# thrill/thrill

Hardware: AMD Instinct MI355X
Metric: TeraSort keys/sec (100-byte recs) (higher is better)
Workload: dtype u8; 1 GPU; terasort_10GiB_100B; records=107374182, record_bytes=100, seed=0x7421, parallelism=dp1

## Files before the change

include/thrill_amd.h:

```cpp
#ifndef THRILL_AMD_H
#define THRILL_AMD_H

#include <stdint.h>

#ifdef __cplusplus
extern "C" {
#endif

typedef struct t9_context t9_context;

int t9_create(t9_context** out, int device, int rank, int world, void* comm);
int t9_destroy(t9_context* ctx);
const char* t9_version(void);

int t9_comm_id_size(void);
int t9_comm_id(void* out_id);
int t9_comm_init(t9_context* ctx, const void* id);

int t9_gen_u64(t9_context* ctx, uint64_t* d_out, uint64_t index0, uint64_t n,
               uint64_t seed, void* stream);
int t9_gen_records(t9_context* ctx, uint8_t* d_out, uint64_t index0,
                   uint64_t n, uint64_t seed, void* stream);


uint64_t t9_sort_u64_workspace(uint64_t n);
int t9_sort_u64(t9_context* ctx, uint64_t* d_keys, uint64_t n,
                void* d_workspace, void* stream);

uint64_t t9_sort_pairs_workspace(uint64_t n);
int t9_sort_pairs_u64_u32(t9_context* ctx, uint64_t* d_keys,
                          uint32_t* d_vals, uint64_t n, void* d_workspace,
                          void* stream);

int t9_extract_key64(t9_context* ctx, const uint8_t* d_recs, uint64_t n,
                     uint32_t rec_size, uint32_t key_off, uint64_t* d_keys,
                     uint32_t* d_idx, void* stream);

int t9_extract_key64_le(t9_context* ctx, const uint8_t* d_recs, uint64_t n,
                        uint32_t rec_size, uint32_t key_off,
                        uint64_t* d_keys, uint32_t* d_idx, void* stream);

int t9_gather_records(t9_context* ctx, const uint8_t* d_recs,
                      const uint32_t* d_idx, uint64_t n, uint32_t rec_size,
                      uint8_t* d_out, void* stream);

uint64_t t9_sort_records_workspace(uint64_t n, uint32_t rec_size);
int t9_sort_records(t9_context* ctx, const uint8_t* d_in, uint8_t* d_out,
                    uint64_t n, uint32_t rec_size, uint32_t key_len,
                    void* d_workspace, void* stream);

int t9_sort_records_keyle(t9_context* ctx, const uint8_t* d_in,
                          uint8_t* d_out, uint64_t n, uint32_t rec_size,
                          void* d_workspace, void* stream);

int t9_sort_last_schedule(const t9_context* ctx);

int t9_sort_last_tiecount(const t9_context* ctx);


int t9_classify_u64(t9_context* ctx, const uint64_t* d_keys, uint64_t n,
                    uint64_t gidx0, const uint64_t* d_spl_keys,
                    const uint64_t* d_spl_idx, uint32_t p,
                    uint32_t* d_bucket, uint64_t* d_counts, void* stream);

int t9_classify_rec(t9_context* ctx, const uint8_t* d_recs,
                    const uint64_t* d_k64, uint64_t n, uint64_t gidx0,
                    const uint8_t* d_spl_recs, const uint64_t* d_spl_k64,
                    const uint64_t* d_spl_idx, uint32_t p, uint32_t rec_size,
                    uint32_t* d_bucket, uint64_t* d_counts, void* stream);

uint64_t t9_partition_idx_workspace(uint64_t n);
int t9_partition_idx(t9_context* ctx, const uint32_t* d_bucket, uint64_t n,
                     uint32_t p, uint32_t* d_perm, uint64_t* d_offsets,
                     void* d_workspace, void* stream);

int t9_alltoall(t9_context* ctx, const void* d_send,
                const uint64_t* send_counts, const uint64_t* send_displs,
                void* d_recv, const uint64_t* recv_counts,
                const uint64_t* recv_displs, uint64_t elem_size,
                void* stream);

int t9_hash_bucket(t9_context* ctx, const uint64_t* d_keys, uint64_t n,
                   uint64_t salt, uint32_t p, uint32_t* d_bucket,
                   uint64_t* d_counts, void* stream);

int t9_reduce_init(t9_context* ctx, uint64_t* d_table, uint64_t capacity,
                   void* stream);
int t9_reduce_build(t9_context* ctx, const uint64_t* d_keys,
                    const uint64_t* d_vals, uint64_t n,
                    uint64_t* d_table, uint64_t capacity, uint64_t salt,
// ... 128 lines not shown
```

thrill_amd/csrc/t9_api.cpp:

```cpp

#include "t9_common.h"

#include <rccl/rccl.h>

#include <cstdlib>
#include <cstring>
#include <new>

extern "C" {

const char* t9_version(void) { return "thrill_amd 0.1 (gfx950)"; }

int t9_create(t9_context** out, int device, int rank, int world,
              void* comm) {
    if (!out || world < 1 || rank < 0 || rank >= world) return T9_EINVAL;
    HIP_TRY(hipSetDevice(device));
    t9_context* ctx = new (std::nothrow) t9_context;
    if (!ctx) return T9_ENOMEM;
    ctx->device = device;
    ctx->rank = rank;
    ctx->world = world;
    ctx->comm = comm;
    ctx->owns_comm = 0;
    ctx->ov_stream = nullptr;
    for (int i = 0; i <= T9_OVERLAP_MAXK; ++i) ctx->ov_ev[i] = nullptr;
    ctx->ov_ready = 0;
    ctx->last_schedule = 0;
    ctx->last_tiecount = 0;
    *out = ctx;
    return T9_OK;
}

int t9_destroy(t9_context* ctx) {
    if (ctx && ctx->comm && ctx->owns_comm)
        ncclCommDestroy((ncclComm_t)ctx->comm);
    if (ctx) {
        if (ctx->ov_stream) {
            (void)hipStreamSynchronize(ctx->ov_stream);
            (void)hipStreamDestroy(ctx->ov_stream);
        }
        for (int i = 0; i <= T9_OVERLAP_MAXK; ++i)
            if (ctx->ov_ev[i]) (void)hipEventDestroy(ctx->ov_ev[i]);
    }
    delete ctx;
    return T9_OK;
}

int t9i_overlap_init(t9_context* ctx) {
    if (!ctx) return T9_EINVAL;
    if (ctx->ov_ready) return T9_OK;
    HIP_TRY(hipSetDevice(ctx->device));
    if (!ctx->ov_stream)
        HIP_TRY(hipStreamCreateWithFlags(&ctx->ov_stream,
                                         hipStreamNonBlocking));
    for (int i = 0; i <= T9_OVERLAP_MAXK; ++i)
        if (!ctx->ov_ev[i])
            HIP_TRY(hipEventCreateWithFlags(&ctx->ov_ev[i],
                                            hipEventDisableTiming));
    ctx->ov_ready = 1;
    return T9_OK;
}

int t9_sort_last_schedule(const t9_context* ctx) {
    return ctx ? ctx->last_schedule : T9_EINVAL;
}

int t9_sort_last_tiecount(const t9_context* ctx) {
    return ctx ? ctx->last_tiecount : T9_EINVAL;
}


int t9_comm_id_size(void) { return (int)sizeof(ncclUniqueId); }

int t9_comm_id(void* out_id) {
    if (!out_id) return T9_EINVAL;
    ncclResult_t rc = ncclGetUniqueId((ncclUniqueId*)out_id);
    if (rc != ncclSuccess) {
        fprintf(stderr, "t9_comm_id: %s\n", ncclGetErrorString(rc));
        return T9_EIO;
    }
    return T9_OK;
}

int t9_comm_init(t9_context* ctx, const void* id) {
    if (!ctx || !id) return T9_EINVAL;
    if (ctx->comm) return T9_EINVAL;
    HIP_TRY(hipSetDevice(ctx->device));
    ncclComm_t comm = nullptr;
    ncclResult_t rc = ncclCommInitRank(&comm, ctx->world,
                                       *(const ncclUniqueId*)id, ctx->rank);
    if (rc != ncclSuccess) {
        fprintf(stderr, "t9_comm_init: rank %d/%d: %s\n", ctx->rank,
                ctx->world, ncclGetErrorString(rc));
        return T9_EIO;
    }
    ctx->comm = comm;
    ctx->owns_comm = 1;
    return T9_OK;
}

int t9_alltoall(t9_context* ctx, const void* d_send, const u64* send_counts,
// ... 58 lines not shown
```

thrill_amd/csrc/t9_bitonic.h:

```cpp
#pragma once
#include "t9_common.h"

__device__ inline void t9_ce_xor(u64& c, u32& v, u32 lanemask, bool lower,
                                 bool asc) {
    const u64 oc = __shfl_xor(c, lanemask);
    const u32 ov = __shfl_xor(v, lanemask);
    if ((c > oc) == (lower == asc)) { c = oc; v = ov; }
}

template <int SUBMAX, int BLOCK, bool HAS_VAL>
__global__ __launch_bounds__(BLOCK, 2) void k_bitonic_sort_sub(
    u64* __restrict__ keys, u32* __restrict__ vals,
    const u32* __restrict__ sub_start, const u32* __restrict__ sub_n) {
    constexpr int E = SUBMAX / BLOCK;
    static_assert(E == 4, "mapping assumes 4 elements per thread");
    __shared__ u64 s_c[SUBMAX];
    __shared__ u32 s_v[HAS_VAL ? SUBMAX : 1];
    __shared__ u32 s_differ;

    const u32 sb = blockIdx.x;
    const u32 ns = sub_n[sb];
    if (ns <= 1 || ns > (u32)SUBMAX) return;
    const u32 gbase = sub_start[sb];
    const u32 tid = threadIdx.x, lane = tid & 63;
// ... 88 lines not shown
        }
    }
}

typedef unsigned long long t9_u64x2 __attribute__((ext_vector_type(2)));

__device__ __forceinline__ u32 t9_w16_phys(u32 e) {
    return e ^ (((e >> 4) & 7u) << 1);
}

__device__ __forceinline__ void t9_w16_row_store(u64* lc, u32 row,
                                                 const u64 (&c)[16]) {
    const u32 base = row * 16 + ((row & 7u) << 1);
#pragma unroll
    for (int k = 0; k < 8; ++k) {
        t9_u64x2 v2;
        v2.x = c[2 * k];
        v2.y = c[2 * k + 1];
        *(t9_u64x2*)&lc[base ^ ((u32)k << 1)] = v2;
    }
}

__device__ __forceinline__ void t9_w16_row_load(const u64* lc, u32 row,
                                                u64 (&c)[16]) {
    const u32 base = row * 16 + ((row & 7u) << 1);
#pragma unroll
    for (int k = 0; k < 8; ++k) {
        const t9_u64x2 v2 = *(const t9_u64x2*)&lc[base ^ ((u32)k << 1)];
        c[2 * k] = v2.x;
        c[2 * k + 1] = v2.y;
    }
}

template <int NSORT, int BLOCK, bool HAS_VAL, bool REC>
__global__ __launch_bounds__(BLOCK, 2) void k_wave16_sort_sub(
    u64* __restrict__ keys, u32* __restrict__ vals,
    const u32* __restrict__ sub_start, const u32* __restrict__ sub_n,
    u32* __restrict__ ntied) {
    constexpr int E = NSORT / BLOCK;
    static_assert(E == 16, "wave16 mapping: 16 elements per lane");
    static_assert(HAS_VAL || !REC, "the tie count rides the pair sort");
    constexpr int ROUNDS = (NSORT == 1024) ? 6 : (NSORT == 2048) ? 7 : 8;
    __shared__ __attribute__((aligned(16))) u64 lc[NSORT];
    __shared__ u32 s_differ;
    __shared__ u32 s_ntie;

    const u32 sb = blockIdx.x;
    const u32 ns = sub_n[sb];
    if (ns <= 1 || ns > (u32)NSORT) return;
    const u32 gbase = sub_start[sb];
    const u32 lane = threadIdx.x;
    const u32 e0 = lane * E;

    if (lane == 0) { s_differ = 0; s_ntie = 0; }
    __syncthreads();

    const u64 mask48 = 0x0000FFFFFFFFFFFFull;
    const u64 high16 = keys[gbase] & ~mask48;
    const u64 ref48 = keys[gbase] & mask48;

    u64 c[E];
    u32 differ = 0;
    u64* const kb = keys + gbase;
    u32* const vb = HAS_VAL ? vals + gbase : nullptr;
#pragma unroll
    for (int r = 0; r < E; ++r) {
        const u32 p = lane + (u32)BLOCK * r;
        u64 cc = ~0ull;
        if (p < ns) {
            const u64 k = kb[p];
            cc = ((k & mask48) << 12) | (u64)p;
            differ |= ((k & mask48) != ref48);
        }
        lc[t9_w16_phys(p)] = cc;
    }
    if (differ) s_differ = 1;
    __syncthreads();
    if (!s_differ) {
        if (REC && lane == 0) atomicAdd(ntied, ns - 1);
        return;
    }
    t9_w16_row_load(lc, lane, c);

#pragma unroll
    for (int lk = 1; lk <= 4; ++lk) {
        const int k = 1 << lk;
#pragma unroll
        for (int lj = lk - 1; lj >= 0; --lj) {
            const int j = 1 << lj;
#pragma unroll
            for (int r = 0; r < E; ++r) {
                const int q = r ^ j;
                if (q > r) {
                    const bool asc = (r & k) == 0;
                    if ((c[r] > c[q]) == asc) {
                        u64 tc = c[r]; c[r] = c[q]; c[q] = tc;
                    }
                }
            }
        }
    }

#pragma unroll
    for (int lm = 0; lm < ROUNDS; ++lm) {
        const u32 L = (u32)E << lm;
        __syncthreads();
        t9_w16_row_store(lc, lane, c);
        __syncthreads();
        const u32 pairbase = e0 & ~(2 * L - 1);
        const u32 d = e0 - pairbase;
        const u32 ab = pairbase, bb = pairbase + L;
        u32 lo = (d > L) ? d - L : 0;
        u32 hi = (d < L) ? d : L;
        while (lo < hi) {
            const u32 m = (lo + hi) >> 1;
            if (lc[t9_w16_phys(ab + m)] <= lc[t9_w16_phys(bb + d - m - 1)])
                lo = m + 1;
            else hi = m;
        }
        u32 ia = ab + lo, ib = bb + (d - lo);
        const u32 ea = bb, eb = bb + L;
        const u64 a0 = lc[t9_w16_phys(ia < ea ? ia : ab)];
        const u64 b0 = lc[t9_w16_phys(ib < eb ? ib : ab)];
        u64 a = (ia < ea) ? a0 : ~0ull;
        u64 b = (ib < eb) ? b0 : ~0ull;
#pragma unroll
        for (int r = 0; r < E; ++r) {
            const bool ta = a <= b;
            c[r] = ta ? a : b;
            if (r + 1 < E) {
                ia += ta ? 1u : 0u;
                ib += ta ? 0u : 1u;
                const u32 nx = ta ? ia : ib;
                const bool in = nx < (ta ? ea : eb);
                const u64 ld = lc[t9_w16_phys(in ? nx : ab)];
                const u64 nv = in ? ld : ~0ull;
                a = ta ? nv : a;
                b = ta ? b : nv;
            }
        }
    }

    __syncthreads();
    t9_w16_row_store(lc, lane, c);
    __syncthreads();
    if (REC) {
        const u64 nxt = (e0 + E < (u32)NSORT) ? lc[t9_w16_phys(e0 + E)]
                                              : ~0ull;
        u32 cnt = 0;
#pragma unroll
        for (int r = 0; r < E; ++r) {
            const u64 hi = (r + 1 < E) ? c[r + 1] : nxt;
            cnt += (e0 + r + 1 < ns) && ((c[r] >> 12) == (hi >> 12));
        }
        if (cnt) atomicAdd(&s_ntie, cnt);
    }
    u32 v[HAS_VAL ? E : 1];
    if (HAS_VAL) {
#pragma unroll
        for (int r = 0; r < E; ++r) {
            const u32 p = lane + (u32)BLOCK * r;
            if (p < ns) v[r] = vb[(u32)lc[t9_w16_phys(p)] & 0xFFFu];
        }
    }
    __syncthreads();
    const u32 nt = REC ? s_ntie : 0u;
    if (REC && lane == 0 && nt) atomicAdd(ntied, nt);
    if (HAS_VAL) {
#pragma unroll
        for (int r = 0; r < E; ++r) {
            const u32 p = lane + (u32)BLOCK * r;
            if (p < ns) vb[p] = v[r];
        }
    }
    if (!REC || nt) {
#pragma unroll
        for (int r = 0; r < E; ++r) {
            const u32 p = lane + (u32)BLOCK * r;
            if (p < ns) kb[p] = high16 | (lc[t9_w16_phys(p)] >> 12);
        }
    }
}

template <int NSORT, int BLOCK, bool HAS_VAL>
__global__ __launch_bounds__(BLOCK, 2) void k_wave16_sort_span(
    const u64* __restrict__ keys_in, const u32* __restrict__ vals_in,
    u64* __restrict__ keys_out, u32* __restrict__ vals_out,
    const u32* __restrict__ span_start, const u32* __restrict__ span_len) {
    constexpr int E = NSORT / BLOCK;
    static_assert(E == 16, "wave16 mapping: 16 elements per lane");
    constexpr int ROUNDS = (NSORT == 1024) ? 6 : (NSORT == 2048) ? 7 : 8;
    __shared__ u64 lc[NSORT];
    __shared__ u32 s_differ;

    const u32 sb = blockIdx.x;
    const u32 ns = span_len[sb];
    if (ns == 0) return;
    const u32 gbase = span_start[sb];
    const u32 lane = threadIdx.x;
    const u32 e0 = lane * E;

    if (ns > (u32)NSORT) {
        if (keys_out != keys_in)
            for (u32 i = lane; i < ns; i += BLOCK) {
                keys_out[gbase + i] = keys_in[gbase + i];
                if (HAS_VAL) vals_out[gbase + i] = vals_in[gbase + i];
            }
        return;
    }

    if (lane == 0) s_differ = 0;
    __syncthreads();
// ... 99 lines not shown
```

thrill_amd/csrc/t9_common.h:

```cpp
#pragma once

#include <hip/hip_runtime.h>
#include <cstdint>
#include <cstdio>

#include "thrill_amd.h"

using u8 = uint8_t;
using u16 = uint16_t;
using u32 = uint32_t;
using u64 = uint64_t;

#define T9_WAVE 64

#define T9_OK 0
#define T9_EINVAL (-22)
#define T9_ENOMEM (-12)
#define T9_EIO (-5)
#define T9_ENOSYS (-38)

#define HIP_TRY(expr)                                                     \
    do {                                                                  \
        hipError_t _e = (expr);                                           \
        if (_e != hipSuccess) {                                           \
            fprintf(stderr, "t9: %s:%d: %s failed: %s\n", __FILE__,       \
                    __LINE__, #expr, hipGetErrorString(_e));              \
            return T9_EIO;                                                \
        }                                                                 \
    } while (0)

#define T9_LAUNCH_CHECK()                                                 \
    do {                                                                  \
        hipError_t _e = hipGetLastError();                                \
        if (_e != hipSuccess) {                                           \
            fprintf(stderr, "t9: %s:%d: kernel launch failed: %s\n",      \
                    __FILE__, __LINE__, hipGetErrorString(_e));           \
            return T9_EIO;                                                \
        }                                                                 \
    } while (0)

#define T9_OVERLAP_MAXK 16

struct t9_context {
    int device;
    int rank;
    int world;
    void* comm;
    int owns_comm;
    hipStream_t ov_stream;
    hipEvent_t ov_ev[T9_OVERLAP_MAXK + 1];
    int ov_ready;
    int last_schedule;
    int last_tiecount;
};

struct t9_overlap_req {
    const u8* recs;
    u8* out;
    u32 rec_words;
    u32 chunks;
};

__host__ __device__ inline u64 t9_splitmix64_at(u64 seed, u64 ctr) {
    u64 z = seed + (ctr + 1) * 0x9E3779B97F4A7C15ull;
    z = (z ^ (z >> 30)) * 0xBF58476D1CE4E5B9ull;
    z = (z ^ (z >> 27)) * 0x94D049BB133111EBull;
    return z ^ (z >> 31);
}

__host__ __device__ inline u64 t9_hash128to64(u64 upper, u64 lower) {
    const u64 k = 0x9DDFEA08EB382D69ull;
    u64 a = (lower ^ upper) * k;
    a ^= (a >> 47);
    u64 b = (upper ^ a) * k;
    b ^= (b >> 47);
    b *= k;
    return b;
}

#define T9_MSB 0x8000000000000000ull

__host__ __device__ inline u64 t9_enc(u64 b, int op, int vtype) {
    if (op == T9_OP_SUM || vtype == T9_VAL_U64) return b;
    if (vtype == T9_VAL_I64) return b ^ T9_MSB;
    return b ^ ((b >> 63) ? ~0ull : T9_MSB);
}
__host__ __device__ inline u64 t9_dec(u64 e, int op, int vtype) {
    if (op == T9_OP_SUM || vtype == T9_VAL_U64) return e;
    if (vtype == T9_VAL_I64) return e ^ T9_MSB;
    return e ^ ((e >> 63) ? T9_MSB : ~0ull);
}

static inline u64 t9_ceil_div(u64 a, u64 b) { return (a + b - 1) / b; }
// ... 18 lines not shown
```

thrill_amd/csrc/t9_records.hip:

```cpp

#include "t9_common.h"
#include "t9_rank_scatter.h"

#include <cstdlib>
#include <cstring>
#include <vector>
#include <algorithm>

extern "C" int t9i_count_tied(const u64* d_keys, u64 n, u32* d_ntied,
                              hipStream_t s);
extern "C" u64 t9_sort_pairs_workspace(u64 n);
extern "C" int t9_sort_pairs_u64_u32(t9_context*, u64*, u32*, u64, void*,
                                     void*);
extern "C" int t9i_sort_recs_msb(t9_context*, const u8*, u32, u64*, u32*,
                                 u64, void*, void*);
extern "C" u64 t9_partition_idx_workspace(u64 n);
extern "C" int t9_partition_idx(t9_context*, const u32*, u64, u32, u32*,
                                u64*, void*, void*);
extern "C" int t9i_sort_pairs_msb_ph(t9_context*, u64*, u32*, u64, void*,
                                     void*, int, t9_overlap_req*, u32*,
                                     int*);
extern "C" u32* t9i_msb_pass1_hist(void* d_workspace, u64 n);


// ... 649 lines not shown
                             void* d_workspace, void* stream, bool le) {
    if (rec_size % 4 || key_len > rec_size || n >= (1ull << 32))
        return T9_EINVAL;
    hipStream_t s = (hipStream_t)stream;
    if (n == 0) return T9_OK;
    if (!d_in || !d_out || !d_workspace) return T9_EINVAL;
    if (d_in == d_out) return T9_EINVAL;
    if (n == 1) {
        HIP_TRY(hipMemcpyAsync(d_out, d_in, rec_size, hipMemcpyDeviceToDevice,
                               s));
        return T9_OK;
    }
    char* p = (char*)d_workspace;
    u64* d_keys = (u64*)p;
    p += t9_align256(n * 8);
    u32* d_idx = (u32*)p;
    p += t9_align256(n * 4);
    void* pair_ws = p;
    p += t9_sort_pairs_workspace(n);
    u32* d_ntied = (u32*)p;

    const char* algo = getenv("T9_SORT_ALGO");
    bool msb_dispatch = n >= (1ull << 22);
    if (algo && strcmp(algo, "lsd") == 0) msb_dispatch = false;
    if (algo && strcmp(algo, "msb") == 0) msb_dispatch = n >= (1ull << 14);
    const char* ehe = getenv("T9_EXTRACT_HIST");
    const u32 rw = rec_size / 4;
    const bool eh = !(ehe && ehe[0] == '0') && msb_dispatch &&
                    (rw == 25 || rw == 32);
    const char* fe = getenv("T9_FUSED_EXTRACT");
    bool fused = fe && atoi(fe) && n >= (1ull << 14) &&
                 (rec_size == 100 || rec_size == 128);
    int rc;
    t9_overlap_req ov = { nullptr, nullptr, 0, 0 };
    int tie_counted = 0;
    if (ctx) { ctx->last_schedule = 0; ctx->last_tiecount = 0; }
    if (eh && !fused) {
        u32* hist = t9i_msb_pass1_hist(pair_ws, n);
        const u64 B = t9_ceil_div(n, 8192);
        const char* sbe = getenv("T9_EXTRACT_SB");
        const bool sb = !(sbe && sbe[0] == '0');
        const char* ie = getenv("T9_EXTRACT_IOTA");
        const bool widx = ie && ie[0] == '1';
        T9_PERF_WRAP(s, "extract",
                     if (widx) launch_extract_hist<true>(
                         rw, le, sb, (u32)B, s, d_in, n, d_keys, d_idx,
                         hist);
                     else launch_extract_hist<false>(
                         rw, le, sb, (u32)B, s, d_in, n, d_keys, d_idx,
                         hist));
        T9_LAUNCH_CHECK();
        const char* gv = getenv("T9_GATHER_VARIANT");
        const bool may_overlap = rw == 25 && ctx && !(gv && atoi(gv) != 3);
        if (may_overlap) {
            ov.recs = d_in;
            ov.out = d_out;
            ov.rec_words = rw;
        }
        rc = t9i_sort_pairs_msb_ph(ctx, d_keys, d_idx, n, pair_ws, stream,
                                   widx ? 0 : 1, may_overlap ? &ov : nullptr,
                                   d_ntied, &tie_counted);
    }
    else if (fused && !le) {
        rc = t9i_sort_recs_msb(ctx, d_in, rec_size, d_keys, d_idx, n,
                               pair_ws, stream);
    }
    else {
        rc = le ? t9_extract_key64_le(ctx, d_in, n, rec_size, 0, d_keys,
                                      d_idx, stream)
                : t9_extract_key64(ctx, d_in, n, rec_size, 0, d_keys,
                                   d_idx, stream);
        if (rc) return rc;
        rc = t9_sort_pairs_u64_u32(ctx, d_keys, d_idx, n, pair_ws, stream);
    }
    if (rc) return rc;
    if (!tie_counted) {
        rc = t9i_count_tied(d_keys, n, d_ntied, s);
        if (rc) return rc;
    }
    if (ctx) ctx->last_tiecount = tie_counted;
    u32 ntied = 0;
    HIP_TRY(hipMemcpyAsync(&ntied, d_ntied, 4, hipMemcpyDeviceToHost, s));
    HIP_TRY(hipStreamSynchronize(s));
    if (ov.chunks) {
        ctx->last_schedule = (int)ov.chunks;
        if (!ntied) return T9_OK;
    }

    if (ntied && rec_size > 8) {
        const u64 need = 6 * t9_align256(n * 4) +
                         2 * t9_align256(n * 8) +
                         t9_align256(3 * 8) + 256 +
                         t9_align256((n / T9_MAXSCAN_TILE + 2) * 4) + 256 +
                         t9_partition_idx_workspace(n);
        void* tmp_alloc = nullptr;
        char* q;
        if ((u64)n * rec_size >= need) {
            q = (char*)d_out;
        }
        else {
            HIP_TRY(hipMalloc(&tmp_alloc, need));
            q = (char*)tmp_alloc;
        }
        u32* t_bucket = (u32*)q; q += t9_align256(n * 4);
        u32* t_perm = (u32*)q;   q += t9_align256(n * 4);
        u32* t_idx = (u32*)q;    q += t9_align256(n * 4);
        u64* t_chunk = (u64*)q;  q += t9_align256(n * 8);
        u64* t_offs = (u64*)q;   q += t9_align256(3 * 8);
        u32* t_flag = (u32*)q;   q += 256;
        u32* t_grp = (u32*)q;    q += t9_align256(n * 4);
        u32* t_grp2 = (u32*)q;   q += t9_align256(n * 4);
        u32* t_tmp4 = (u32*)q;   q += t9_align256(n * 4);
        u64* t_chunk2 = (u64*)q; q += t9_align256(n * 8);
        u32* t_part = (u32*)q;
        q += t9_align256((n / T9_MAXSCAN_TILE + 2) * 4);
        u32* t_ties = (u32*)q;   q += 256;
        void* t_pws = q;

// ... 164 lines not shown
```

thrill_amd/csrc/t9_sort_msb.hip:

```cpp

#include "t9_common.h"
#include "t9_rank_scatter.h"
#include "t9_bitonic.h"

#include <cstdlib>
#include <vector>

#define T9_MSB_TILE 8192
#define T9_SUBMAX 4096
#define T9_MSB_MIN (1u << 22)

__global__ void k_colsum(const u32*, u64, u32*);
__global__ void k_chunkscan(u32*, u64, u32*);
__global__ void k_finaloffs(u32*, u64, const u32*, const u32*);
__global__ void k_grp_scan(u32*, u64, u64*);

extern "C" void t9i_launch_hist_seg9(u32, void*, const u64*, const u32*,
                                     const u32*, u32*);
extern "C" void t9i_launch_seg_scan9(u32, void*, u32*, const u32*,
                                     const u32*, const u32*, u32*, u32*);
extern "C" void t9i_launch_scatter_seg9(u32, int, void*, const u64*,
                                        const u32*, const u32*, const u32*,
                                        u64*, u32*, const u32*);
constexpr u64 NSUB9 = 256ull * 512;
// ... 892 lines not shown
    u64 l3 = 0;
    if (n >= T9_L3_MIN || (l3e && atoi(l3e) == 3))
        l3 = t9_align256((u64)(NSUB + 1) * 4) + 256 +
             2 * t9_align256(NSUB3 * 4) +
             t9_align256((2 * (NSUB3 + 64) + 1) * 4);
    return l3 + t9_align256(npad * 8) + t9_align256(npad * 4) +
           t9_align256(B2max * T9_RADIX * 4) +
           t9_align256(t9_ceil_div(B2max, T9_SCAN_CHUNK) * T9_RADIX * 4) +
           4 * t9_align256(T9_RADIX * 4) + t9_align256(257 * 4) +
           2 * t9_align256(NSUB9 * 4) +
           t9_align256((u64)(NSUB + 2) * 4) +
           t9_align256((u64)(2 * (NSUB + 64) + 1) * 4);
}
}

extern "C" u64 t9i_sort_pairs_msb_workspace(u64 n) { return msb_ws_bytes(n); }

extern "C" int t9i_overlap_init(t9_context* ctx);
extern "C" int t9i_gather_chunk(const u8*, const u32*, u64, u64, u8*,
                                const u32*, hipStream_t);

#define T9_OVERLAP_K 8

static u32 overlap_chunks() {
    const char* on = getenv("T9_SORT_OVERLAP");
    if (!on || on[0] == '0' || on[0] == '\0') return 0;
    const char* e = getenv("T9_SORT_OVERLAP_CHUNKS");
    int k = e ? atoi(e) : T9_OVERLAP_K;
    if (k < 1) k = 1;
    if (k > T9_OVERLAP_MAXK) k = T9_OVERLAP_MAXK;
    return (u32)k;
}

__global__ __launch_bounds__(64) void k_chunk_bounds(
    const u32* __restrict__ sub_start, u32 nsub, u32 K,
    const u32* __restrict__ info, u32* __restrict__ out) {
    const u32 c = threadIdx.x;
    if (c < 2) out[c] = info[c];
    if (c >= 1 && c < K)
        out[1 + c] = sub_start[(u64)c * nsub / K];
}

template <bool HAS_VAL, int RW = 0>
static int sort_msb_impl(t9_context* ctx, const u64* pass1_src,
                         u64* d_keys, u32* d_vals, u64 n,
                         void* d_workspace, void* stream,
                         bool pre_hist = false,
                         t9_overlap_req* ov = nullptr,
                         bool iota_vals = false,
                         u32* d_ntied = nullptr,
                         int* tie_counted = nullptr) {
    hipStream_t s = (hipStream_t)stream;
    MsbWs w = carve_msb((char*)d_workspace, n);

    {
        const u64 B = w.B1;
        const u64 Bc = t9_ceil_div(B, T9_SCAN_CHUNK);
        if (!pre_hist)
            T9_PERF_WRAP(s, "hist_pairs",
                         hipLaunchKernelGGL((k_hist_msb<RW>), dim3((u32)B),
                                            dim3(256), 0, s, pass1_src, n,
                                            56, w.hist));
        hipLaunchKernelGGL(k_colsum, dim3((u32)Bc), dim3(256), 0, s, w.hist,
                           B, w.chunkpart);
        hipLaunchKernelGGL(k_chunkscan, dim3(1), dim3(256), 0, s,
                           w.chunkpart, Bc, w.digit_base);
// ... 72 lines not shown
                bnd[K] = n;
                bool mono = true;
                for (u32 c = 1; c < K; ++c) {
                    bnd[c] = info[1 + c];
                    mono = mono && bnd[c] >= bnd[c - 1] && bnd[c] <= n;
                }
                if (mono) {
                    int rc = t9i_overlap_init(ctx);
                    if (rc) return rc;
                    hipStream_t sb = ctx->ov_stream;
                    u32 done = 0;
                    for (u32 c = 0; c < K; ++c) {
                        const u64 a = bnd[c], b = bnd[c + 1];
                        if (a == b) continue;
                        const u32 sub0 = (u32)((u64)c * NSUB9 / K);
                        const u32 sub1 = (u32)((u64)(c + 1) * NSUB9 / K);
                        t9i_launch_wave16_sub<HAS_VAL>(
                            sub1 - sub0, maxsub, s, d_keys, d_vals,
                            w.sub_start + sub0, w.sub_n + sub0, tcount);
                        T9_LAUNCH_CHECK();
                        HIP_TRY(hipEventRecord(ctx->ov_ev[c], s));
                        HIP_TRY(hipStreamWaitEvent(sb, ctx->ov_ev[c], 0));
                        rc = t9i_gather_chunk(
                            ov->recs, d_vals + a, b - a, n,
                            ov->out + a * (u64)ov->rec_words * 4,
                            tcount, sb);
                        if (rc) return rc;
                        ++done;
                    }
                    HIP_TRY(hipEventRecord(ctx->ov_ev[T9_OVERLAP_MAXK], sb));
                    HIP_TRY(hipStreamWaitEvent(
                        s, ctx->ov_ev[T9_OVERLAP_MAXK], 0));
                    ov->chunks = done;
                    return T9_OK;
                }
            }
            T9_PERF_WRAP(
                s, "lds_sort",
                if (t9i_lds_wave16() && maxsub <= t9i_wave16_max())
                    t9i_launch_wave16_sub<HAS_VAL>((u32)NSUB9, maxsub, s,
                                                   d_keys, d_vals,
                                                   w.sub_start, w.sub_n,
                                                   tcount);
                else if (t9i_lds_bitonic())
                    t9i_launch_bitonic_sub<HAS_VAL>((u32)NSUB9, maxsub, s,
                                                    d_keys, d_vals,
                                                    w.sub_start, w.sub_n);
                else if (maxsub <= 1024)
                    hipLaunchKernelGGL(
                        (k_lds_sort_sub<1024, 256, HAS_VAL>), dim3(NSUB9),
                        dim3(256), 0, s, d_keys, d_vals, w.sub_start,
                        w.sub_n);
                else if (maxsub <= 2048)
                    hipLaunchKernelGGL(
                        (k_lds_sort_sub<2048, 512, HAS_VAL>), dim3(NSUB9),
                        dim3(512), 0, s, d_keys, d_vals, w.sub_start,
                        w.sub_n);
                else
                    hipLaunchKernelGGL(
                        (k_lds_sort_sub<T9_SUBMAX, 1024, HAS_VAL>),
                        dim3(NSUB9), dim3(1024), 0, s, d_keys, d_vals,
                        w.sub_start, w.sub_n));
            T9_LAUNCH_CHECK();
            if (novr9 == 0) return T9_OK;
            if (novr9 > 64)
                return HAS_VAL ? t9i_sort_pairs_lsd(ctx, d_keys, d_vals, n,
// ... 292 lines not shown
```

thrill_amd/native.py:

```python
import ctypes
import os

HERE = os.path.dirname(os.path.abspath(__file__))
SO = os.path.join(HERE, "libt9.so")

u64 = ctypes.c_uint64
u32 = ctypes.c_uint32
i32 = ctypes.c_int
vp = ctypes.c_void_p


T9_OP_SUM, T9_OP_MIN, T9_OP_MAX = 0, 1, 2
T9_VAL_U64, T9_VAL_I64, T9_VAL_F64 = 0, 1, 2
T9_EINVAL = -22


class T9Error(RuntimeError):
    pass


def lib_path():
    return SO


def load_lib(path=None):
    path = path or SO
    if not os.path.exists(path):
        raise T9Error(
            f"libt9.so not found at {path}; build it with "
            "`make -C thrill_amd` (hipcc --offload-arch=gfx950). "
            "There is no CPU fallback.")
    return ctypes.CDLL(path)


_SIGS = {
    "t9_version": (ctypes.c_char_p, []),
    "t9_create": (i32, [ctypes.POINTER(vp), i32, i32, i32, vp]),
    "t9_destroy": (i32, [vp]),
    "t9_comm_id_size": (i32, []),
    "t9_comm_id": (i32, [vp]),
    "t9_comm_init": (i32, [vp, vp]),
    "t9_gen_u64": (i32, [vp, vp, u64, u64, u64, vp]),
    "t9_gen_records": (i32, [vp, vp, u64, u64, u64, vp]),
    "t9_sort_u64_workspace": (u64, [u64]),
    "t9_sort_u64": (i32, [vp, vp, u64, vp, vp]),
    "t9_sort_pairs_workspace": (u64, [u64]),
    "t9_sort_pairs_u64_u32": (i32, [vp, vp, vp, u64, vp, vp]),
    "t9_extract_key64": (i32, [vp, vp, u64, u32, u32, vp, vp, vp]),
    "t9_gather_records": (i32, [vp, vp, vp, u64, u32, vp, vp]),
    "t9_sort_records_workspace": (u64, [u64, u32]),
    "t9_sort_records": (i32, [vp, vp, vp, u64, u32, u32, vp, vp]),
    "t9_sort_records_keyle": (i32, [vp, vp, vp, u64, u32, vp, vp]),
    "t9_sort_last_schedule": (i32, [vp]),
    "t9_sort_last_tiecount": (i32, [vp]),
    "t9_extract_key64_le": (i32, [vp, vp, u64, u32, u32, vp, vp, vp]),
    "t9_classify_u64": (i32, [vp, vp, u64, u64, vp, vp, u32, vp, vp, vp]),
    "t9_classify_rec": (i32, [vp, vp, vp, u64, u64, vp, vp, vp, u32, u32,
                              vp, vp, vp]),
    "t9_partition_idx_workspace": (u64, [u64]),
    "t9_partition_idx": (i32, [vp, vp, u64, u32, vp, vp, vp, vp]),
    "t9_alltoall": (i32, [vp, vp, vp, vp, vp, vp, vp, u64, vp]),
    "t9_hash_bucket": (i32, [vp, vp, u64, u64, u32, vp, vp, vp]),
    "t9_reduce_by_index": (i32, [vp, vp, vp, u64, u64, u64, vp, vp, vp]),
    "t9_index_bucket": (i32, [vp, vp, u64, u64, u64, u32, vp, vp, vp, vp]),
    "t9_reduce_init": (i32, [vp, vp, u64, vp]),
    "t9_reduce_build": (i32, [vp, vp, vp, u64, vp, u64, u64, vp, vp]),
    "t9_reduce_drain": (i32, [vp, vp, u64, vp, vp, vp, vp]),
    "t9_reduce128_table_words": (u64, [u64]),
    "t9_reduce128_init": (i32, [vp, vp, u64, vp]),
    "t9_reduce128_build": (i32, [vp, vp, vp, vp, u64, vp, u64, u64, vp,
                                 vp]),
    "t9_reduce128_drain": (i32, [vp, vp, u64, vp, vp, vp, vp, vp]),
    "t9_reduce128_lookup": (i32, [vp, vp, vp, u64, vp, u64, u64, vp, vp]),
    "t9_hash2_of": (i32, [vp, vp, u64, vp, vp, vp]),
    "t9_reduce_init_op": (i32, [vp, vp, u64, i32, i32, vp]),
    "t9_reduce_build_op": (i32, [vp, vp, vp, u64, vp, u64, u64, i32, i32,
                                 vp, vp]),
    "t9_reduce_drain_op": (i32, [vp, vp, u64, i32, i32, vp, vp, vp, vp]),
    "t9_reduce128_init_op": (i32, [vp, vp, u64, i32, i32, vp]),
    "t9_reduce128_build_op": (i32, [vp, vp, vp, vp, u64, vp, u64, u64, i32,
                                    i32, vp, vp]),
    "t9_reduce128_drain_op": (i32, [vp, vp, u64, i32, i32, vp, vp, vp, vp,
                                    vp]),
    "t9_reduce_by_index_op_workspace": (u64, [u64]),
    "t9_reduce_by_index_op": (i32, [vp, vp, vp, u64, u64, u64, i32, i32,
                                    u64, vp, vp, vp, vp]),
    "t9_scan_geometry": (None, [ctypes.POINTER(u32), ctypes.POINTER(u32)]),
# ... 41 lines not shown
        def call(*args):
            rc = fn(self.ctx, *args)
            if rc != 0:
                raise T9Error(f"t9_{name} failed rc={rc}")
            return rc
        return call

    def comm_id(self):
        size = self._lib.t9_comm_id_size()
        buf = (ctypes.c_uint8 * size)()
        rc = self._lib.t9_comm_id(buf)
        if rc != 0:
            raise T9Error(f"t9_comm_id failed rc={rc}")
        return bytes(buf)

    def comm_init(self, id_bytes):
        buf = (ctypes.c_uint8 * len(id_bytes)).from_buffer_copy(id_bytes)
        rc = self._lib.t9_comm_init(self.ctx, buf)
        if rc != 0:
            raise T9Error(f"t9_comm_init failed rc={rc}")

    def sort_last_schedule(self):
        k = self._lib.t9_sort_last_schedule(self.ctx)
        if k < 0:
            raise T9Error(f"t9_sort_last_schedule failed rc={k}")
        return k

    def sort_last_tiecount(self):
        k = self._lib.t9_sort_last_tiecount(self.ctx)
        if k < 0:
            raise T9Error(f"t9_sort_last_tiecount failed rc={k}")
        return k

    def perf_enable(self, on):
        self._lib.t9_perf_enable(1 if on else 0)

    def perf_read(self, cls):
        ms = ctypes.c_double()
        n = u64()
        rc = self._lib.t9_perf_read(cls.encode(), ctypes.byref(ms),
                                    ctypes.byref(n))
        if rc != 0:
            raise T9Error(f"t9_perf_read failed rc={rc}")
        return ms.value, n.value

    def perf_reset(self):
        self._lib.t9_perf_reset()

    def ws(self, name, *args):
        return getattr(self._lib, f"t9_{name}_workspace")(*args)

    def reduce128_table_words(self, capacity):
        return self._lib.t9_reduce128_table_words(capacity)

    def scan_geometry(self):
        t, p = u32(), u32()
        self._lib.t9_scan_geometry(ctypes.byref(t), ctypes.byref(p))
        return t.value, p.value

    def version(self):
        return self._lib.t9_version().decode()

    def close(self):
        if self.ctx:
            self._lib.t9_destroy(self.ctx)
            self.ctx = None
# ... 1 lines not shown
```

Before: 8.898 billion keys/s.

## Fuse subbucket sort with tie resolution and record gather in one kernel

Adds a kernel that sorts each small subbucket by its 48-bit key suffix, resolves short runs of tied keys by comparing the remaining record bytes, and then gathers the 100-byte records straight into the output. This is enabled by default when no overlap chunking is in use. The aim is to remove the separate gather pass and the re-read of keys and indices between the sort and the gather. If any subbucket has unresolved ties, a global counter suppresses the fused gather and execution falls back to the old path. That adds serial tail comparisons and an atomic-flag dependency between blocks.

```diff
diff --git a/include/thrill_amd.h b/include/thrill_amd.h
--- a/include/thrill_amd.h
+++ b/include/thrill_amd.h
@@ -56,6 +56,8 @@
 int t9_sort_last_schedule(const t9_context* ctx);
 
 int t9_sort_last_tiecount(const t9_context* ctx);
+
+int t9_sort_last_fused(const t9_context* ctx);
 
 
 int t9_classify_u64(t9_context* ctx, const uint64_t* d_keys, uint64_t n,
diff --git a/thrill_amd/csrc/t9_api.cpp b/thrill_amd/csrc/t9_api.cpp
--- a/thrill_amd/csrc/t9_api.cpp
+++ b/thrill_amd/csrc/t9_api.cpp
@@ -27,6 +27,7 @@
     ctx->ov_ready = 0;
     ctx->last_schedule = 0;
     ctx->last_tiecount = 0;
+    ctx->last_fused = 0;
     *out = ctx;
     return T9_OK;
 }
@@ -67,6 +68,10 @@
 
 int t9_sort_last_tiecount(const t9_context* ctx) {
     return ctx ? ctx->last_tiecount : T9_EINVAL;
+}
+
+int t9_sort_last_fused(const t9_context* ctx) {
+    return ctx ? ctx->last_fused : T9_EINVAL;
 }
 
 
diff --git a/thrill_amd/csrc/t9_bitonic.h b/thrill_amd/csrc/t9_bitonic.h
--- a/thrill_amd/csrc/t9_bitonic.h
+++ b/thrill_amd/csrc/t9_bitonic.h
@@ -144,56 +144,10 @@
     }
 }
 
-template <int NSORT, int BLOCK, bool HAS_VAL, bool REC>
-__global__ __launch_bounds__(BLOCK, 2) void k_wave16_sort_sub(
-    u64* __restrict__ keys, u32* __restrict__ vals,
-    const u32* __restrict__ sub_start, const u32* __restrict__ sub_n,
-    u32* __restrict__ ntied) {
-    constexpr int E = NSORT / BLOCK;
-    static_assert(E == 16, "wave16 mapping: 16 elements per lane");
-    static_assert(HAS_VAL || !REC, "the tie count rides the pair sort");
-    constexpr int ROUNDS = (NSORT == 1024) ? 6 : (NSORT == 2048) ? 7 : 8;
-    __shared__ __attribute__((aligned(16))) u64 lc[NSORT];
-    __shared__ u32 s_differ;
-    __shared__ u32 s_ntie;
-
-    const u32 sb = blockIdx.x;
-    const u32 ns = sub_n[sb];
-    if (ns <= 1 || ns > (u32)NSORT) return;
-    const u32 gbase = sub_start[sb];
-    const u32 lane = threadIdx.x;
+template <int E, int ROUNDS>
+__device__ __forceinline__ void t9_w16_blocksort(u64* lc, u32 lane,
+                                                 u64 (&c)[E]) {
     const u32 e0 = lane * E;
-
-    if (lane == 0) { s_differ = 0; s_ntie = 0; }
-    __syncthreads();
-
-    const u64 mask48 = 0x0000FFFFFFFFFFFFull;
-    const u64 high16 = keys[gbase] & ~mask48;
-    const u64 ref48 = keys[gbase] & mask48;
-
-    u64 c[E];
-    u32 differ = 0;
-    u64* const kb = keys + gbase;
-    u32* const vb = HAS_VAL ? vals + gbase : nullptr;
-#pragma unroll
-    for (int r = 0; r < E; ++r) {
-        const u32 p = lane + (u32)BLOCK * r;
-        u64 cc = ~0ull;
-        if (p < ns) {
-            const u64 k = kb[p];
-            cc = ((k & mask48) << 12) | (u64)p;
-            differ |= ((k & mask48) != ref48);
-        }
-        lc[t9_w16_phys(p)] = cc;
-    }
-    if (differ) s_differ = 1;
-    __syncthreads();
-    if (!s_differ) {
-        if (REC && lane == 0) atomicAdd(ntied, ns - 1);
-        return;
-    }
-    t9_w16_row_load(lc, lane, c);
-
 #pragma unroll
     for (int lk = 1; lk <= 4; ++lk) {
         const int k = 1 << lk;
@@ -252,6 +206,116 @@
             }
         }
     }
+}
+
+template <int NSORT, int BLOCK, bool HAS_VAL, bool REC>
+__global__ __launch_bounds__(BLOCK, 2) void k_wave16_sort_sub(
+    u64* __restrict__ keys, u32* __restrict__ vals,
+    const u32* __restrict__ sub_start, const u32* __restrict__ sub_n,
+    u32* __restrict__ ntied) {
+    constexpr int E = NSORT / BLOCK;
+    static_assert(E == 16, "wave16 mapping: 16 elements per lane");
+    static_assert(HAS_VAL || !REC, "the tie count rides the pair sort");
+    constexpr int ROUNDS = (NSORT == 1024) ? 6 : (NSORT == 2048) ? 7 : 8;
+    __shared__ __attribute__((aligned(16))) u64 lc[NSORT];
+    __shared__ u32 s_differ;
+    __shared__ u32 s_ntie;
+
+    const u32 sb = blockIdx.x;
+    const u32 ns = sub_n[sb];
+    if (ns <= 1 || ns > (u32)NSORT) return;
+    const u32 gbase = sub_start[sb];
+    const u32 lane = threadIdx.x;
+    const u32 e0 = lane * E;
+
+    if (lane == 0) { s_differ = 0; s_ntie = 0; }
+    __syncthreads();
+
+    const u64 mask48 = 0x0000FFFFFFFFFFFFull;
+    const u64 high16 = keys[gbase] & ~mask48;
+    const u64 ref48 = keys[gbase] & mask48;
+
+    u64 c[E];
+    u32 differ = 0;
+    u64* const kb = keys + gbase;
+    u32* const vb = HAS_VAL ? vals + gbase : nullptr;
+#pragma unroll
+    for (int r = 0; r < E; ++r) {
+        const u32 p = lane + (u32)BLOCK * r;
+        u64 cc = ~0ull;
+        if (p < ns) {
+            const u64 k = kb[p];
+            cc = ((k & mask48) << 12) | (u64)p;
+            differ |= ((k & mask48) != ref48);
+        }
+        lc[t9_w16_phys(p)] = cc;
+    }
+    if (differ) s_differ = 1;
+    __syncthreads();
+    if (!s_differ) {
+        if (REC && lane == 0) atomicAdd(ntied, ns - 1);
+        return;
+    }
+    t9_w16_row_load(lc, lane, c);
+
+#pragma unroll
+    for (int lk = 1; lk <= 4; ++lk) {
+        const int k = 1 << lk;
+#pragma unroll
+        for (int lj = lk - 1; lj >= 0; --lj) {
+            const int j = 1 << lj;
+#pragma unroll
+            for (int r = 0; r < E; ++r) {
+                const int q = r ^ j;
+                if (q > r) {
+                    const bool asc = (r & k) == 0;
+                    if ((c[r] > c[q]) == asc) {
+                        u64 tc = c[r]; c[r] = c[q]; c[q] = tc;
+                    }
+                }
+            }
+        }
+    }
+
+#pragma unroll
+    for (int lm = 0; lm < ROUNDS; ++lm) {
+        const u32 L = (u32)E << lm;
+        __syncthreads();
+        t9_w16_row_store(lc, lane, c);
+        __syncthreads();
+        const u32 pairbase = e0 & ~(2 * L - 1);
+        const u32 d = e0 - pairbase;
+        const u32 ab = pairbase, bb = pairbase + L;
+        u32 lo = (d > L) ? d - L : 0;
+        u32 hi = (d < L) ? d : L;
+        while (lo < hi) {
+            const u32 m = (lo + hi) >> 1;
+            if (lc[t9_w16_phys(ab + m)] <= lc[t9_w16_phys(bb + d - m - 1)])
+                lo = m + 1;
+            else hi = m;
+        }
+        u32 ia = ab + lo, ib = bb + (d - lo);
+        const u32 ea = bb, eb = bb + L;
+        const u64 a0 = lc[t9_w16_phys(ia < ea ? ia : ab)];
+        const u64 b0 = lc[t9_w16_phys(ib < eb ? ib : ab)];
+        u64 a = (ia < ea) ? a0 : ~0ull;
+        u64 b = (ib < eb) ? b0 : ~0ull;
+#pragma unroll
+        for (int r = 0; r < E; ++r) {
+            const bool ta = a <= b;
+            c[r] = ta ? a : b;
+            if (r + 1 < E) {
+                ia += ta ? 1u : 0u;
+                ib += ta ? 0u : 1u;
+                const u32 nx = ta ? ia : ib;
+                const bool in = nx < (ta ? ea : eb);
+                const u64 ld = lc[t9_w16_phys(in ? nx : ab)];
+                const u64 nv = in ? ld : ~0ull;
+                a = ta ? nv : a;
+                b = ta ? b : nv;
+            }
+        }
+    }
 
     __syncthreads();
     t9_w16_row_store(lc, lane, c);
@@ -290,6 +354,186 @@
         for (int r = 0; r < E; ++r) {
             const u32 p = lane + (u32)BLOCK * r;
             if (p < ns) kb[p] = high16 | (lc[t9_w16_phys(p)] >> 12);
+        }
+    }
+}
+
+#define T9_FUSED_RUNMAX 8
+
+__device__ __forceinline__ bool t9_rec100_tail_less(
+    const u32* __restrict__ rin, u32 ra, u32 rb) {
+    const u32* a = rin + (u64)ra * 25;
+    const u32* b = rin + (u64)rb * 25;
+#pragma unroll 1
+    for (int w = 2; w < 25; ++w) {
+        const u32 x = __builtin_bswap32(a[w]), y = __builtin_bswap32(b[w]);
+        if (x != y) return x < y;
+    }
+    return false;
+}
+
+template <int D, bool TIES>
+__global__ __launch_bounds__(64, 2) void k_wave16_sort_gather(
+    u64* __restrict__ keys, u32* __restrict__ vals,
+    const u32* __restrict__ sub_start, const u32* __restrict__ sub_n,
+    u32* ntied, const u32* __restrict__ rin, u32* __restrict__ rout) {
+    constexpr int NSORT = 1024, BLOCK = 64, E = 16, ROUNDS = 6, RW = 25;
+    __shared__ __attribute__((aligned(16))) u64 lc[NSORT];
+    __shared__ u32 s_differ;
+    __shared__ u32 s_ntie;
+    __shared__ u32 s_settled;
+
+    const u32 sb = blockIdx.x;
+    const u32 ns = sub_n[sb];
+    if (ns == 0 || ns > (u32)NSORT) return;
+    const u32 gbase = sub_start[sb];
+    const u32 lane = threadIdx.x;
+    const u32 e0 = lane * E;
+    u32* const ob = rout + (u64)gbase * RW;
+
+    if (ns == 1) {
+        if (__hip_atomic_load(ntied, __ATOMIC_RELAXED,
+                              __HIP_MEMORY_SCOPE_AGENT))
+            return;
+        if (lane < (u32)RW) ob[lane] = rin[(u64)vals[gbase] * RW + lane];
+        return;
+    }
+
+    if (lane == 0) { s_differ = 0; s_ntie = 0; s_settled = 0; }
+    __syncthreads();
+
+    const u64 mask48 = 0x0000FFFFFFFFFFFFull;
+    const u64 high16 = keys[gbase] & ~mask48;
+    const u64 ref48 = keys[gbase] & mask48;
+
+    u64 c[E];
+    u32 differ = 0;
+    u64* const kb = keys + gbase;
+    u32* const vb = vals + gbase;
+#pragma unroll
+    for (int r = 0; r < E; ++r) {
+        const u32 p = lane + (u32)BLOCK * r;
+        u64 cc = ~0ull;
+        if (p < ns) {
+            const u64 k = kb[p];
+            cc = ((k & mask48) << 12) | (u64)p;
+            differ |= ((k & mask48) != ref48);
+        }
+        lc[t9_w16_phys(p)] = cc;
+    }
+    if (differ) s_differ = 1;
+    __syncthreads();
+    if (!s_differ) {
+        if (lane == 0) atomicAdd(ntied, ns - 1);
+        return;
+    }
+    t9_w16_row_load(lc, lane, c);
+
+    t9_w16_blocksort<E, ROUNDS>(lc, lane, c);
+
+    __syncthreads();
+    t9_w16_row_store(lc, lane, c);
+    __syncthreads();
+    {
+        const u64 nxt = (e0 + E < (u32)NSORT) ? lc[t9_w16_phys(e0 + E)]
+                                              : ~0ull;
+        u32 cnt = 0;
+#pragma unroll
+        for (int r = 0; r < E; ++r) {
+            const u64 hi = (r + 1 < E) ? c[r + 1] : nxt;
+            cnt += (e0 + r + 1 < ns) && ((c[r] >> 12) == (hi >> 12));
+        }
+        if (cnt) atomicAdd(&s_ntie, cnt);
+    }
+    __syncthreads();
+    const u32 nt = s_ntie;
+    if (TIES && nt) {
+        u32 settled = 0;
+#pragma unroll 1
+        for (u32 e = e0; e < e0 + E && e + 1 < ns; ++e) {
+            const u64 key = lc[t9_w16_phys(e)] >> 12;
+            if ((lc[t9_w16_phys(e + 1)] >> 12) != key) continue;
+            if (e > 0 && (lc[t9_w16_phys(e - 1)] >> 12) == key) continue;
+            u32 len = 2;
+            while (len <= T9_FUSED_RUNMAX && e + len < ns &&
+                   (lc[t9_w16_phys(e + len)] >> 12) == key)
+                ++len;
+            if (len > T9_FUSED_RUNMAX) continue;
+            for (u32 i = 1; i < len; ++i)
+                for (u32 j = i; j > 0; --j) {
+                    const u32 hi_at = t9_w16_phys(e + j);
+                    const u32 lo_at = t9_w16_phys(e + j - 1);
+                    const u64 ch = lc[hi_at], cl = lc[lo_at];
+                    const u32 ph = (u32)ch & 0xFFFu, pl = (u32)cl & 0xFFFu;
+                    if (!t9_rec100_tail_less(rin, vb[ph], vb[pl])) break;
+                    lc[hi_at] = (ch & ~0xFFFull) | pl;
+                    lc[lo_at] = (cl & ~0xFFFull) | ph;
+                }
+            settled += len - 1;
+        }
+        if (settled) atomicAdd(&s_settled, settled);
+    }
+    __syncthreads();
+    u32 v[E];
+#pragma unroll
+    for (int r = 0; r < E; ++r) {
+        const u32 p = lane + (u32)BLOCK * r;
+        if (p < ns) v[r] = vb[(u32)lc[t9_w16_phys(p)] & 0xFFFu];
+    }
+    __syncthreads();
+    const u32 unsettled = nt - s_settled;
+    if (lane == 0 && unsettled) atomicAdd(ntied, unsettled);
+#pragma unroll
+    for (int r = 0; r < E; ++r) {
+        const u32 p = lane + (u32)BLOCK * r;
+        if (p < ns) vb[p] = v[r];
+    }
+    if (nt) {
+#pragma unroll
+        for (int r = 0; r < E; ++r) {
+            const u32 p = lane + (u32)BLOCK * r;
+            if (p < ns) kb[p] = high16 | (lc[t9_w16_phys(p)] >> 12);
+        }
+    }
+    if (unsettled) return;
+
+    __syncthreads();
+    u32* const li = (u32*)lc;
+#pragma unroll
+    for (int r = 0; r < E; ++r) {
+        const u32 p = lane + (u32)BLOCK * r;
+        if (p < ns) li[p] = v[r];
+    }
+    __syncthreads();
+    if (__hip_atomic_load(ntied, __ATOMIC_RELAXED, __HIP_MEMORY_SCOPE_AGENT))
+        return;
+    const u32 W = ns * RW;
+    for (u32 g0 = lane; g0 < W; g0 += (u32)BLOCK * D) {
+        u32 x[D];
+        if (g0 - lane + (u32)BLOCK * D <= W) {
+#pragma unroll
+            for (int j = 0; j < D; ++j) {
+                const u32 g = g0 + (u32)BLOCK * j;
+                const u32 rec = g / (u32)RW;
+                x[j] = rin[(u64)li[rec] * RW + (g - rec * RW)];
+            }
+#pragma unroll
+            for (int j = 0; j < D; ++j) ob[g0 + (u32)BLOCK * j] = x[j];
+        }
+        else {
+#pragma unroll
+            for (int j = 0; j < D; ++j) {
+                const u32 g = g0 + (u32)BLOCK * j;
+                if (g < W) {
+                    const u32 rec = g / (u32)RW;
+                    x[j] = rin[(u64)li[rec] * RW + (g - rec * RW)];
+                }
+            }
+#pragma unroll
+            for (int j = 0; j < D; ++j) {
+                const u32 g = g0 + (u32)BLOCK * j;
+                if (g < W) ob[g] = x[j];
+            }
         }
     }
 }
diff --git a/thrill_amd/csrc/t9_common.h b/thrill_amd/csrc/t9_common.h
--- a/thrill_amd/csrc/t9_common.h
+++ b/thrill_amd/csrc/t9_common.h
@@ -52,6 +52,7 @@
     int ov_ready;
     int last_schedule;
     int last_tiecount;
+    int last_fused;
 };
 
 struct t9_overlap_req {
@@ -59,6 +60,7 @@
     u8* out;
     u32 rec_words;
     u32 chunks;
+    u32 fused;
 };
 
 __host__ __device__ inline u64 t9_splitmix64_at(u64 seed, u64 ctr) {
diff --git a/thrill_amd/csrc/t9_records.hip b/thrill_amd/csrc/t9_records.hip
--- a/thrill_amd/csrc/t9_records.hip
+++ b/thrill_amd/csrc/t9_records.hip
@@ -705,9 +705,13 @@
     bool fused = fe && atoi(fe) && n >= (1ull << 14) &&
                  (rec_size == 100 || rec_size == 128);
     int rc;
-    t9_overlap_req ov = { nullptr, nullptr, 0, 0 };
+    t9_overlap_req ov = { nullptr, nullptr, 0, 0, 0 };
     int tie_counted = 0;
-    if (ctx) { ctx->last_schedule = 0; ctx->last_tiecount = 0; }
+    if (ctx) {
+        ctx->last_schedule = 0;
+        ctx->last_tiecount = 0;
+        ctx->last_fused = 0;
+    }
     if (eh && !fused) {
         u32* hist = t9i_msb_pass1_hist(pair_ws, n);
         const u64 B = t9_ceil_div(n, 8192);
@@ -757,6 +761,10 @@
     HIP_TRY(hipStreamSynchronize(s));
     if (ov.chunks) {
         ctx->last_schedule = (int)ov.chunks;
+        if (!ntied) return T9_OK;
+    }
+    if (ov.fused) {
+        ctx->last_fused = ntied ? 2 : 1;
         if (!ntied) return T9_OK;
     }
 
diff --git a/thrill_amd/csrc/t9_sort_msb.hip b/thrill_amd/csrc/t9_sort_msb.hip
--- a/thrill_amd/csrc/t9_sort_msb.hip
+++ b/thrill_amd/csrc/t9_sort_msb.hip
@@ -948,6 +948,22 @@
     return (u32)k;
 }
 
+#ifndef T9_FUSED_D
+#define T9_FUSED_D 16
+#endif
+#ifndef T9_FUSED_TIES
+#define T9_FUSED_TIES 1
+#endif
+#ifndef T9_FUSED_DEFAULT
+#define T9_FUSED_DEFAULT 1
+#endif
+
+static bool t9i_fused_gather() {
+    const char* e = getenv("T9_SORT_FUSED_GATHER");
+    if (!e || e[0] == '\0') return T9_FUSED_DEFAULT != 0;
+    return e[0] != '0';
+}
+
 __global__ __launch_bounds__(64) void k_chunk_bounds(
     const u32* __restrict__ sub_start, u32 nsub, u32 K,
     const u32* __restrict__ info, u32* __restrict__ out) {
@@ -1086,6 +1102,20 @@
                     HIP_TRY(hipStreamWaitEvent(
                         s, ctx->ov_ev[T9_OVERLAP_MAXK], 0));
                     ov->chunks = done;
+                    return T9_OK;
+                }
+            }
+            if constexpr (HAS_VAL) {
+                if (tcount && ov && ctx && !t9perf_on() && ov->recs &&
+                    ov->rec_words == 25 && overlap_chunks() == 0 &&
+                    maxsub <= 1024 && t9i_fused_gather()) {
+                    hipLaunchKernelGGL(
+                        (k_wave16_sort_gather<T9_FUSED_D, T9_FUSED_TIES != 0>),
+                        dim3((u32)NSUB9), dim3(64), 0, s, d_keys, d_vals,
+                        w.sub_start, w.sub_n, tcount, (const u32*)ov->recs,
+                        (u32*)ov->out);
+                    T9_LAUNCH_CHECK();
+                    ov->fused = 1;
                     return T9_OK;
                 }
             }
diff --git a/thrill_amd/native.py b/thrill_amd/native.py
--- a/thrill_amd/native.py
+++ b/thrill_amd/native.py
@@ -53,6 +53,7 @@
     "t9_sort_records_keyle": (i32, [vp, vp, vp, u64, u32, vp, vp]),
     "t9_sort_last_schedule": (i32, [vp]),
     "t9_sort_last_tiecount": (i32, [vp]),
+    "t9_sort_last_fused": (i32, [vp]),
     "t9_extract_key64_le": (i32, [vp, vp, u64, u32, u32, vp, vp, vp]),
     "t9_classify_u64": (i32, [vp, vp, u64, u64, vp, vp, u32, vp, vp, vp]),
     "t9_classify_rec": (i32, [vp, vp, vp, u64, u64, vp, vp, vp, u32, u32,
@@ -160,6 +161,12 @@
             raise T9Error(f"t9_sort_last_tiecount failed rc={k}")
         return k
 
+    def sort_last_fused(self):
+        k = self._lib.t9_sort_last_fused(self.ctx)
+        if k < 0:
+            raise T9Error(f"t9_sort_last_fused failed rc={k}")
+        return k
+
     def perf_enable(self, on):
         self._lib.t9_perf_enable(1 if on else 0)
 
```

After: 9.289 billion keys/s (median of 6 runs). 1.04x the previous value.
